# scheckmedia/centernet-uda

Hardware: AMD Instinct MI355X
Metric: images/sec CenterNet DLA-34 512x512 UDA step (entropy minimisation) (higher is better)
Workload: dtype f32; 1 GPU; configs[2]: DLA-34 + DCNv2, 512x512, per-GPU batch 16 source + 16 target, uda=entropy_minimization, Adam(lr 5e-5), random-init weights; global_batch=16, parallelism=dp1

## Files before the change

### centernet-uda_amd/csrc/conv.hip

```cpp
#include <stdlib.h>

#include <type_traits>
#include <algorithm>
#include "igemm.cuh"
#include "hconv.cuh"
#include "hwgrad.cuh"
#include "igemm_host.h"

namespace cnuda {
namespace {

struct ConvGeom {
    int B, C, H, W, Co, kh, kw, sh, sw, ph, pw, Ho, Wo;
};

struct ConvFwdParams {
    ConvGeom g;
    const float *x, *bias;
    float* y;
    float act_slope;
    const float* residual;
};
struct ConvFwdStatsParams : ConvFwdParams {
    float* stats;
// ... 1111 lines not shown
                                 : (ws ? "igemm_fwd_ws_kernel<%d, %s>" : "igemm_fwd_kernel<%d, %s>"), bm, Loader::name());
    if (matrix_mode() == 1) {
        float* A3 = const_cast<float*>(A) + (size_t)Kp * Mp;
        CNUDA_LAUNCH(split_a_kernel, dim3(stream_grid((long long)(Kp / 16) * 2 * Mp, 256)), dim3(256), 0, st, A,
                           reinterpret_cast<u32x4*>(A3), Kp, Mp);
        found = with_tile<32, 64, 128>(bm, [&](auto BM) {
            CNUDA_LAUNCH((igemm_fwd_kernel<BM(), Loader, true>), grid, block, 0, st, p, A3, Mp, Kp, M, N, n_tiles, m_tiles);
        });
    } else if (ws) {
        found = with_tile<64, 128>(bm, [&](auto BM) {
            CNUDA_LAUNCH((igemm_fwd_ws_kernel<BM(), Loader>), grid, block2, 0, st, p, A, Mp, Kp, M, N, n_tiles, m_tiles);
        });
    } else {
        found = with_tile<32, 64, 128>(bm, [&](auto BM) {
            CNUDA_LAUNCH((igemm_fwd_kernel<BM(), Loader>), grid, block, 0, st, p, A, Mp, Kp, M, N, n_tiles, m_tiles);
        });
    }
    CNUDA_REQUIRE(found, "%s: no igemm_fwd kernel instance for a %d-row tile", who, bm);
    return check_launch(who);
}

template <class Loader>
bool launch_wgrad_buf(const ConvPlan& q, const typename Loader::Params& p, float* slabs, float* bsl, hipStream_t st) {
    return q.wgrad_ws ? launch_wgrad<Loader, true, Tile<128, 128>, Tile<128, 64>, Tile<64, 128>, Tile<64, 64>>(q.wg, p, slabs, bsl, st)
                      : launch_wgrad<Loader, false, Tile<128, 128>, Tile<128, 64>, Tile<64, 128>, Tile<64, 64>, Tile<32, 128>>(q.wg, p, slabs, bsl, st);
}

using PlanQuery = bool (*)(const ConvGeom&, const ConvPlan&);
bool plan_cat_ok(const ConvGeom& g, const ConvPlan& q) {
    return q.fwd == FwdPath::Buf && q.dgrad == DgradPath::Buf && q.wgrad == WgradPath::Buf && ((g.H * g.W) & 3) == 0;
}
bool plan_rowquads_ok(const ConvGeom& g, const ConvPlan& q) { return g.Co % 4 == 0 && q.fwd != FwdPath::SmallC && q.fwd != FwdPath::BufSplitK && q.fwd_buf; }
bool plan_rowsig_ok(const ConvGeom& g, const ConvPlan& q) { return g.Co <= 32 && matrix_mode() == 0 && q.fwd != FwdPath::SmallC && q.fwd_buf && q.y_buf; }
int plan_query(PlanQuery ok, const char* who, int B, int C, int H, int W, int Co, int kh, int kw, int sh, int sw, int ph, int pw) {
    ConvGeom g;
    if (fill_geom(g, B, C, H, W, Co, kh, kw, sh, sw, ph, pw, who)) return 0;
    return ok(g, make_plan(g)) ? 1 : 0;
}

enum class ConvDir { Fwd = 0, Dgrad = 1, Wgrad = 2 };
struct ConvCall {
    const char* who;
    hipStream_t st;
    void* workspace;  size_t workspace_bytes;
    Carver cv;
    bool gemm_only = false;
    ConvGeom g;
    ConvPlan q;
    ConvCall(const char* who_, void* ws, size_t bytes, cnuda_stream_t stream)
        : who(who_), st((hipStream_t)stream), workspace(ws), workspace_bytes(bytes), cv(ws, bytes) {}
    FwdPath fwd() const { return gemm_only ? q.fwd_gemm : q.fwd; }
    DgradPath dgrad() const { return gemm_only ? q.dgrad_gemm : q.dgrad; }
    int open(ConvDir dir, bool gemm_only_, int B, int C, int H, int W, int Co, int kh, int kw, int sh, int sw, int ph, int pw,
             PlanQuery ok = nullptr, const char* unsupported = nullptr) {
        gemm_only = gemm_only_;
        const int bad = fill_geom(g, B, C, H, W, Co, kh, kw, sh, sw, ph, pw, who);
        if (!bad) q = make_plan(g);
        if (ok) CNUDA_REQUIRE(!bad && ok(g, q), "%s: %s", who, unsupported);
        if (bad) return bad;
        const bool lds_tiles[] = {fwd() == FwdPath::SmallC, dgrad() == DgradPath::SmallC, q.wgrad == WgradPath::SmallC};
        const size_t need[] = {q.fwd_bytes, q.dgrad_bytes, q.wgrad_bytes};
        CNUDA_REQUIRE(lds_tiles[(int)dir] || (workspace && workspace_bytes >= need[(int)dir]), "%s: workspace too small", who);
        return 0;
    }
    void rewind() { cv = Carver(workspace, workspace_bytes); }
    float* a_room(int Kp, int Mp) { return reinterpret_cast<float*>(cv.take<char>(ig_a_bytes(Kp, Mp))); }
// ... 182 lines not shown
}

extern "C" int cnuda_conv2d_forward_res(const float* x, const float* weight, const float* bias, const float* residual,
                                        float* y, int B, int C, int H, int W, int Cout, int kh, int kw, int sh, int sw,
                                        int ph, int pw, float act_slope, void* workspace, size_t workspace_bytes,
                                        cnuda_stream_t stream) {
    return cnuda_conv2d_forward_stats(x, weight, bias, residual, y, nullptr, B, C, H, W, Cout, kh, kw, sh, sw, ph, pw, act_slope,
                                      workspace, workspace_bytes, stream);
}

extern "C" int cnuda_conv2d_forward_stats(const float* x, const float* weight, const float* bias, const float* residual,
                                          float* y, float* stats, int B, int C, int H, int W, int Cout, int kh, int kw,
                                          int sh, int sw, int ph, int pw, float act_slope, void* workspace,
                                          size_t workspace_bytes, cnuda_stream_t stream) {
    CNUDA_REQUIRE(x && weight && y, "cnuda_conv2d_forward: null pointer");
    ConvCall c("cnuda_conv2d_forward", workspace, workspace_bytes, stream);
    if (int rc = c.open(ConvDir::Fwd, residual != nullptr, B, C, H, W, Cout, kh, kw, sh, sw, ph, pw)) return rc;
    CNUDA_REQUIRE(!stats || (!residual && act_slope < 0.0f && plan_stats_block(c.g, c.q, nullptr, nullptr) != 0),
                  "cnuda_conv2d_forward_stats: no statistics for this call (cnuda_conv2d_stats_block says which)");
    if (c.fwd() == FwdPath::SmallC)
        return smallc_forward(x, weight, bias, y, B, C, H, W, Cout, kh, kw, sh, ph, pw, act_slope, 0, workspace,
                              workspace_bytes, c.st, stats);
    ConvFwdParams p{c.g, x, bias, y, act_slope, residual};
    const float* A = c.pack(weight, c.fwd() == FwdPath::Halo ? PACK_HALO_FWD : PACK_FWD);
    switch (c.fwd()) {
        case FwdPath::Halo: return launch_hconv<HconvFwd>(c.q.bmf, p, x, C, c.g, A, c.q.Mpf, c.q.Kpf, Cout, c.q.Nf, c.st, c.who);
        case FwdPath::BufSplitK: case FwdPath::Buf:
            if (stats)
                return c.fwd_gemm<ConvFwdBufStatsLoader>(ConvFwdStatsParams{p, stats, c.q.Mpf}, A, "cnuda_conv2d_forward_stats");
            return c.fwd_gemm<ConvFwdBufLoader>(p, A, c.who, c.q.skf, c.splitk_slabs(c.q.skf, Cout, c.q.Nf));
        case FwdPath::PtrFast: return c.fwd_gemm<ConvFwdLoader<true>>(p, A, c.who);
        default: return c.fwd_gemm<ConvFwdLoader<false>>(p, A, c.who);
    }
}

extern "C" int cnuda_conv2d_cat_supported(const int* cs, int n, int B, int H, int W, int Cout) {
    const int C = cat_channels(cs, n);
    return C > 0 ? plan_query(plan_cat_ok, "cnuda_conv2d_cat_supported", B, C, H, W, Cout, 1, 1, 1, 1, 0, 0) : 0;
}

extern "C" int cnuda_conv2d_cat_forward(const float* const* xs, const int* cs, int n, const float* weight, const float* bias,
                                        float* y, float* stats, float act_slope, int B, int H, int W, int Cout,
                                        void* workspace, size_t workspace_bytes, cnuda_stream_t stream) {
    CNUDA_REQUIRE(weight && y, "cnuda_conv2d_cat_forward: null pointer");
    CNUDA_REQUIRE(!stats || act_slope < 0.0f, "cnuda_conv2d_cat_forward: statistics are those of the plain convolution");
    ConvCall c("cnuda_conv2d_cat_forward", workspace, workspace_bytes, stream);
    if (int rc = open_cat(c, ConvDir::Fwd, cs, n, B, H, W, Cout)) return rc;
    ConvFwdCatParams p{{{c.g, nullptr, bias, y, act_slope, nullptr}, stats, c.q.Mpf}, {}};
    if (int rc = fill_cat(p.cat, xs, cs, n, c.who)) return rc;
    return c.fwd_gemm<ConvFwdCatLoader>(p, c.pack(weight, PACK_FWD), c.who);
}

extern "C" int cnuda_conv2d_cat_backward_data(const float* grad_y, const float* weight, float* const* grad_xs,
                                              const float* const* adds, const float* const* add2s, const int* cs, int n,
                                              int B, int H, int W, int Cout, void* workspace, size_t workspace_bytes,
                                              cnuda_stream_t stream) {
    CNUDA_REQUIRE(grad_y && weight && grad_xs, "cnuda_conv2d_cat_backward_data: null pointer");
    ConvCall c("cnuda_conv2d_cat_backward_data", workspace, workspace_bytes, stream);
    if (int rc = open_cat(c, ConvDir::Dgrad, cs, n, B, H, W, Cout)) return rc;
    const float* A = c.pack(weight, PACK_DGRAD);
    ConvDgradCatParams p{{c.g, grad_y, nullptr, round_up(Cout, IG_BK), nullptr, nullptr}};
    for (int i = 0; i < CAT_MAX; ++i) {
        p.gxs[i] = i < n ? grad_xs[i] : nullptr;
        p.adds[i] = (i < n && adds) ? adds[i] : nullptr;
        p.add2s[i] = (i < n && add2s) ? add2s[i] : nullptr;
        if (!p.adds[i] && p.add2s[i]) { p.adds[i] = p.add2s[i]; p.add2s[i] = nullptr; }
// ... 179 lines not shown
```

### centernet-uda_amd/csrc/igemm.cuh

```cuda
#pragma once
#include <type_traits>
#include <utility>
#include "common.h"
#include "igemm_host.h"

namespace cnuda {

using f32x16 = __attribute__((ext_vector_type(16))) float;

constexpr int IG_BN = 128;
constexpr int IG_BK = 16;
constexpr int IG_KC = 16;
constexpr int IG_THREADS = 256;

template <int BM> struct IgTile;
template <> struct IgTile<128> { static constexpr int WM = 2, WN = 2, TM = 2, TN = 2; };
template <> struct IgTile<64>  { static constexpr int WM = 2, WN = 2, TM = 1, TN = 2; };
template <> struct IgTile<32>  { static constexpr int WM = 1, WN = 4, TM = 1, TN = 1; };

__device__ __forceinline__ int xcd_remap(int bid, int nwg) {
    constexpr int NX = 8;
    const int per = nwg / NX, rem = nwg % NX;
    const int x = bid % NX, q = bid / NX;
    const int start = x * per + (x < rem ? x : rem);
// ... 571 lines not shown
    }
    if constexpr (Loader::Out::kVec4) {
        if (Loader::Out::vec4_ok(p)) {
            ig_epilogue_vec4<BM, Loader>(p, smem + wid * IG_EPI_WAVE, acc, m0, n0, wm_off, wn_off, lane, M, N);
            return;
        }
    }
#pragma unroll
    for (int j = 0; j < T::TN; ++j) {
        const long long n = n0 + wn_off + j * 32 + (lane & 31);
        if (n >= N) continue;
        typename Loader::Out out(p, n);
#pragma unroll
        for (int i = 0; i < T::TM; ++i)
#pragma unroll
            for (int r = 0; r < 16; ++r) {
                const int m = m0 + wm_off + i * 32 + mfma_row(r, lane);
                if (m < M) out.store(p, m, acc[i][j][r]);
            }
    }
}

template <int BM, class Loader, int KC = IG_KC>
__global__ __launch_bounds__(2 * IG_THREADS, (BM == 128 ? 2 : 1)) void igemm_fwd_ws_kernel(
    typename Loader::Params p, const float* __restrict__ A, int Mp, int Kp, int M, long long N,
    int n_tiles, int m_tiles) {
    igemm_fwd_ws_body<BM, Loader, KC>(p, A, Mp, Kp, M, N, n_tiles, m_tiles);
}
template <int BM, class Loader, int KC = IG_KC>
__global__ __launch_bounds__(2 * IG_THREADS, (BM == 128 ? 2 : 1)) void igemm_fwd_ws_splitk_kernel(
    typename Loader::Params p, const float* __restrict__ A, int Mp, int Kp, int M, long long N,
    int n_tiles, int m_tiles, float* __restrict__ slab, int split_k) {
    igemm_fwd_ws_body<BM, Loader, KC, true>(p, A, Mp, Kp, M, N, n_tiles, m_tiles, slab, split_k);
}

template <int BMT, int LDA, class Loader, int KP>
__device__ __forceinline__ void ig_shortk_tile(const typename Loader::Params& p, float* __restrict__ As,
                                               const float* __restrict__ Bs, int m0, long long n0, int lane, int wid, int M,
                                               long long N) {
    using T = IgTile<BMT>;
    const int wm_off = (wid / T::WN) * (T::TM * 32), wn_off = (wid % T::WN) * (T::TN * 32);
    f32x16 acc[T::TM][T::TN];
    ig_zero(acc);
#pragma unroll
    for (int c = 0; c < KP / IG_KC; ++c)
        ig_mma_chunk<BMT, IG_KC, LDA>(As + c * IG_KC * LDA, Bs + c * IG_KC * IG_BN, acc, wm_off, wn_off, lane);
    if constexpr (IgHasQuads<typename Loader::Out>::value) {
        ig_epilogue_quads<BMT, Loader>(p, acc, m0, n0, wm_off, wn_off, lane, M, N);
        return;
    }
    __syncthreads();
    if constexpr (Loader::Out::kVec4) {
        if (Loader::Out::vec4_ok(p)) {
            ig_epilogue_vec4<BMT, Loader>(p, As + wid * IG_EPI_WAVE, acc, m0, n0, wm_off, wn_off, lane, M, N);
            return;
        }
    }
#pragma unroll
    for (int j = 0; j < T::TN; ++j) {
        const long long n = n0 + wn_off + j * 32 + (lane & 31);
        if (n >= N) continue;
        typename Loader::Out out(p, n);
#pragma unroll
        for (int i = 0; i < T::TM; ++i)
#pragma unroll
            for (int r = 0; r < 16; ++r) {
// ... 309 lines not shown
```

### centernet-uda_amd/hip_runtime/__init__.py

```python
import ctypes
import os
import threading
import weakref

import torch

_PKG_ROOT = os.path.dirname(os.path.dirname(os.path.abspath(__file__)))
LIB_PATH = os.path.join(_PKG_ROOT, 'libcenternet_uda_hip.so')
ABI_VERSION = 2

_lib = None
_lock = threading.Lock()
_workspaces = {}

c_int, c_size_t, c_void_p, c_float = ctypes.c_int, ctypes.c_size_t, ctypes.c_void_p, ctypes.c_float


def lib():
    global _lib
    if _lib is None:
        with _lock:
            if _lib is None:
                if not os.path.exists(LIB_PATH):
                    raise RuntimeError(
# ... 27 lines not shown
class _Sig:
    cnuda_decode_workspace_bytes = (c_size_t, [_I] * 5)
    cnuda_decode_set_max_bands = (_I, [_I])
    cnuda_decode_set_stage2_threads = (_I, [_I])
    cnuda_decode_detection = (_I, [_P] * 5 + [_I] * 8 + _WS)
    cnuda_nms = (_I, [_P, _P] + [_I] * 5 + [_P])
    cnuda_dcn_v2_workspace_bytes = (c_size_t, [_I] * 14)
    cnuda_dcn_v2_forward = (_I, [_P] * 6 + [_I] * 14 + _WS)
    cnuda_dcn_v2_backward = (_I, [_P] * 11 + [_I] * 14 + _WS)
    cnuda_dcn_v2_forward_cols = (_I, [_P] * 7 + [_I] * 14 + _WS)
    cnuda_dcn_v2_forward_act = (_I, [_P] * 7 + [_F] + [_I] * 14 + _WS)
    cnuda_dcn_v2_forward_stats = (_I, [_P] * 8 + [_I] * 16 + _WS)
    cnuda_dcn_v2_stats_block = (_I, [_I] * 14 + [_P])
    cnuda_dcn_v2_forward_om = (_I, [_P] * 7 + [_I] * 2 + [_F] + [_I] * 14 + _WS)
    cnuda_dcn_v2_backward_om = (_I, [_P] * 7 + [_I] + [_P] * 3 + [_I] * 14 + _WS)
    cnuda_dcn_v2_backward_cols = (_I, [_P] * 12 + [_I] * 14 + _WS)
    cnuda_dcn_v2_backward_acc = (_I, [_P] * 8 + [_I] + [_P] * 4 + [_I] * 14 + _WS)
    cnuda_dcn_v2_psroi_pooling_workspace_bytes = (c_size_t, [_I] * 4)
    cnuda_dcn_v2_psroi_pooling_forward = (_I, [_P] * 5 + [_I] * 6 + [_F] + [_I] * 5 + [_F, _I, _P])
    cnuda_dcn_v2_psroi_pooling_backward = (_I, [_P] * 6 + [_I, _P] + [_I] * 6 + [_F] + [_I] * 5 + [_F, _I] + _WS)
    cnuda_eval_workspace_bytes = (c_size_t, [_I, _I])
    cnuda_eval_box_spans = (_I, [_P, _I, _I, _I, _P, _P] + _WS)
    cnuda_eval_iou_rotated = (_I, [_P, _I, _I, _I, _LL, _P, _P, _I, _P] + _WS)
    cnuda_eval_iou_axis = (_I, [_P, _P, _P, _I, _I, _I, _LL, _P, _P])
    cnuda_eval_iou_quads = (_I, [_P, _P, _I, _I, _I, _LL, _P, _P, _P])
    cnuda_eval_match = (_I, [_P, _P, _I, _P, _P, _I, _I, _LL, _P, _I, _P, _P, _P, _P])
    cnuda_eval_match_flagged = (_I, [_P, _P, _I, _P, _P, _P, _I, _I, _LL, _P, _I, _P, _P, _P, _P])
    cnuda_eval_oks = (_I, [_P] * 6 + [_I, _P, _I, _I, _I, _LL, _P, _P, _P, _P])
    cnuda_conv2d_workspace_bytes = (c_size_t, [_I] * 11)
    cnuda_conv2d_forward = (_I, [_P] * 4 + [_I] * 11 + [_F] + _WS)
    cnuda_conv2d_forward_res = (_I, [_P] * 5 + [_I] * 11 + [_F] + _WS)
    cnuda_conv2d_rowsig_supported = (_I, [_I] * 11)
    cnuda_conv2d_forward_rowsig = (_I, [_P] * 4 + [_I] * 12 + _WS)
    cnuda_conv2d_rowquads_supported = (_I, [_I] * 11)
    cnuda_conv2d_cat_supported = (_I, [_P, _I, _I, _I, _I, _I])
    cnuda_conv2d_cat_forward = (_I, [_P, _P, _I, _P, _P, _P, _P, _F, _I, _I, _I, _I] + _WS)
    cnuda_conv2d_cat_backward_data = (_I, [_P, _P, _P, _P, _P, _P, _I, _I, _I, _I, _I] + _WS)
    cnuda_conv2d_cat_backward_weight = (_I, [_P, _P, _I, _P, _P, _I, _I, _I, _I] + _WS)
    cnuda_conv2d_forward_rowquads = (_I, [_P] * 3 + [_I] * 11 + _WS)
    cnuda_conv2d_backward_data = (_I, [_P] * 3 + [_I] * 11 + _WS)
    cnuda_conv2d_backward_data_add = (_I, [_P] * 5 + [_I] * 11 + _WS)
    cnuda_conv2d_stats_block = (_I, [_I] * 11 + [_P, _P])
    cnuda_conv2d_forward_stats = (_I, [_P] * 6 + [_I] * 11 + [_F] + _WS)
    cnuda_bn_train_forward_stats = (_I, [_P, _P, _LL, _I] + [_P] * 9 + [_F, _F, _I, _I, _I, _LL, _I] + _WS)
    cnuda_conv2d_backward_weight = (_I, [_P] * 4 + [_I] * 11 + _WS)
    cnuda_conv2d_norm_input_supported = (_I, [_I] * 11)
    cnuda_conv2d_forward_norm_input = (_I, [_P] * 5 + [_I] + [_P] * 4 + [_I] * 11 + [_F] + _WS)
    cnuda_conv2d_backward_weight_norm_input = (_I, [_P] * 5 + [_I] + [_P] * 3 + [_I] * 11 + _WS)
    cnuda_bn_workspace_bytes = (c_size_t, [_I, _I, _LL])
    cnuda_bn_plan = (_I, [_I, _I, _LL, _I] + [_P] * 4)
    cnuda_bn_train_forward = (_I, [_P] * 10 + [_F, _F, _I, _I, _I, _LL, _I] + _WS)
    cnuda_bn_eval_forward = (_I, [_P] * 7 + [_F, _I, _I, _I, _LL, _P])
    cnuda_bn_backward = (_I, [_P] * 11 + [_I, _I, _I, _LL, _I] + _WS)
    cnuda_maxpool2d_forward = (_I, [_P] * 2 + [_I] * 5 + [_P])
    cnuda_maxpool2d_backward = (_I, [_P] * 3 + [_I] * 5 + [_P])
    cnuda_maxpool2d_backward_acc = (_I, [_P] * 3 + [_I] * 6 + [_P])
    cnuda_maxpool2d_window_forward = (_I, [_P] * 2 + [_I] * 7 + [_P])
    cnuda_maxpool2d_window_backward = (_I, [_P] * 3 + [_I] * 7 + [_P])
    cnuda_dwconvt2d_forward = (_I, [_P] * 3 + [_I] * 7 + [_P])
    cnuda_dwconvt2d_add_forward = (_I, [_P] * 4 + [_I] * 7 + [_P])
    cnuda_dwconvt2d_workspace_bytes = (c_size_t, [_I] * 3)
    cnuda_dwconvt2d_backward = (_I, [_P] * 5 + [_I] * 7 + _WS)
    cnuda_dwconv2d_workspace_bytes = (c_size_t, [_I] * 3)
    cnuda_dwconv2d_forward = (_I, [_P] * 3 + [_I] * 7 + [_P])
    cnuda_dwconv2d_backward = (_I, [_P] * 5 + [_I] * 7 + _WS)
    cnuda_dwconv2d_same_workspace_bytes = (c_size_t, [_I] * 3)
# ... 457 lines not shown
```

### centernet-uda_amd/hip_runtime/nn.py

```python
import math

import torch
from torch import nn

from . import ops


def _pair(v):
    return tuple(v) if isinstance(v, (tuple, list)) else (v, v)


class Conv2d(nn.Module):

    def __init__(self, in_channels, out_channels, kernel_size, stride=1, padding=0, bias=True, act_slope=-1.0,
                 emit_stats=False):
        super().__init__()
        self.in_channels, self.out_channels = in_channels, out_channels
        self.kernel_size, self.stride, self.padding = _pair(kernel_size), _pair(stride), _pair(padding)
        self.act_slope = float(act_slope)
        self.emit_stats = bool(emit_stats)
        self.weight = nn.Parameter(torch.empty(out_channels, in_channels, *self.kernel_size))
        self.bias = nn.Parameter(torch.empty(out_channels)) if bias else None
        from . import PackToken
        self._pack_token = PackToken()
# ... 38 lines not shown
                                  defer_apply=self.defer_apply and self.training)


class MaxPool2d(nn.Module):
    def __init__(self, kernel_size, stride=None, padding=0):
        super().__init__()
        self.kernel_size = int(kernel_size)
        self.stride = self.kernel_size if stride is None else int(stride)
        self.padding = int(padding)

    def forward(self, x):
        return ops.max_pool2d(x, self.kernel_size, self.stride, self.padding)


class ConvTranspose2d(nn.Module):

    def __init__(self, in_channels, out_channels, kernel_size, stride=1, padding=0, output_padding=0):
        super().__init__()
        self.in_channels, self.out_channels = in_channels, out_channels
        self.kernel_size, self.stride = _pair(kernel_size), _pair(stride)
        self.padding, self.output_padding = _pair(padding), _pair(output_padding)
        self.weight = nn.Parameter(torch.empty(in_channels, out_channels, *self.kernel_size))
        bound = 1.0 / math.sqrt(out_channels * self.kernel_size[0] * self.kernel_size[1])
        with torch.no_grad():
            self.weight.uniform_(-bound, bound)

    def forward(self, x):
        return ops.conv_transpose2d(x, self.weight, self.stride, self.padding, self.output_padding)


class Head(nn.Sequential):

    def forward(self, x, lead=None):
        if len(self) == 3 and isinstance(self[0], Conv2d) and isinstance(self[2], Conv2d) \
                and not any(m._forward_hooks or m._forward_pre_hooks for m in self) \
                and (x.requires_grad or any(p.requires_grad for p in self.parameters())) \
                and ops.conv_act_conv1x1_supported(x, self[0], self[2]):
            return ops.conv_act_conv1x1(x, self[0], self[2], lead)
        return super().forward(x if lead is None else x[:lead])


class DepthwiseConvTranspose2d(nn.Module):

    def __init__(self, channels, kernel_size, stride, padding):
        super().__init__()
        self.channels, self.kernel_size, self.stride, self.padding = channels, kernel_size, stride, padding
        self.weight = nn.Parameter(torch.empty(channels, 1, kernel_size, kernel_size))
        with torch.no_grad():
            self.weight.uniform_(-1.0 / kernel_size, 1.0 / kernel_size)

    def forward(self, x, skip=None):
        return ops.depthwise_conv_transpose2d(x, self.weight, self.stride, self.padding, skip)


class DepthwiseConv2d(nn.Module):

    def __init__(self, channels, kernel_size, stride=1, padding=0):
        super().__init__()
        self.channels, self.kernel_size, self.stride, self.padding = channels, kernel_size, stride, padding
        self.in_channels = self.out_channels = channels
        self.weight = nn.Parameter(torch.empty(channels, 1, kernel_size, kernel_size))
        with torch.no_grad():
            self.weight.uniform_(-1.0 / kernel_size, 1.0 / kernel_size)

    def forward(self, x):
        return ops.depthwise_conv2d(x, self.weight, self.stride, self.padding)


class DepthwiseConv2dSame(nn.Module):

    def __init__(self, channels, kernel_size, stride=1, image_size=None):
# ... 98 lines not shown
```

### centernet-uda_amd/hip_runtime/ops.py

```python
import ctypes
import os

import torch
from torch.autograd import Function
from torch.autograd.function import once_differentiable

from . import check, f32c, lib, pack_stamp, prof_arm, ptr, require_gpu, stats_side_output, stream, workspace
from .arena import grad_sink
from .fanout import accumulate_in_place, accumulate_target, claim, first_writer, slot_of


def _pair(v):
    return tuple(v) if isinstance(v, (tuple, list)) else (v, v)


def _ws(nbytes, like):
    w = workspace(nbytes, like.device)
    return ptr(w), w.numel()


def _param_grad(param, needed=True):
    if not needed or param is None:
        return None, None
    v = grad_sink(param)
# ... 106 lines not shown
    if bias is None or not lib().cnuda_conv2d_rowsig_supported(*g):
        return None
    return _Conv2d.apply(x, weight, bias, stride, padding, -1.0, pack_token, None, None, int(sig_from))


EPILOGUE_STATS = True


def with_bn_stats(emit, call):
    if not (emit and EPILOGUE_STATS):
        return call(None)
    box = []
    y = call(box)
    if box:
        y._cnuda_bn_stats = box[0]
    return y


def conv2d(x, weight, bias=None, stride=1, padding=0, act_slope=-1.0, pack_token=0, emit_stats=False):
    norm = getattr(x, '_cnuda_deferred_bn', None)
    if norm is not None:
        g = _conv_geom(x, weight, stride, padding)
        if not lib().cnuda_conv2d_norm_input_supported(*g):
            raise RuntimeError("conv2d: the input is a deferred BatchNorm output, but no apply-on-load kernel takes this "
                               "convolution (cnuda_conv2d_norm_input_supported); ask batch_norm_act to apply it")
    return with_bn_stats(emit_stats, lambda box: _Conv2d.apply(x, weight, bias, stride, padding, float(act_slope), pack_token,
                                                               box, norm, None))


HEAD_SPARSE = os.environ.get('CNUDA_HEAD_SPARSE', '1') != '0'
HEAD_SPARSE_RATIO = 40


def _mark_sparse_rows(grad, ind, mask, B, M, HW):
    grad._cnuda_sparse_rows = (ind, mask, B, M, HW, grad._version)


def _sparse_rows_of(gy, B, HW):
    mark = gy.__dict__.pop('_cnuda_sparse_rows', None)
    if mark is None or mark[5] != gy._version or mark[2] != B or mark[4] != HW or not gy.is_contiguous():
        return None
    return mark[0], mark[1], mark[3]


class _ConvActConv1x1(Function):

    @staticmethod
    def forward(ctx, x, w1, b1, w2, b2, padding, act_slope, token1, token2, lead=None):
        require_gpu(x, w1, b1, w2, b2)
        ctx.slot, ctx.full = slot_of(x), None
        if lead is not None and lead < x.shape[0]:
            ctx.full = x.shape
            x = f32c(x)[:lead]
        x, w1, w2 = f32c(x), f32c(w1), f32c(w2)
        b1 = None if b1 is None else f32c(b1)
        b2 = None if b2 is None else f32c(b2)
        g1 = _conv_geom(x, w1, 1, padding)
        hidden = _conv_forward(g1, x, w1, b1, act_slope, token1)
        g2 = _conv_geom(hidden, w2, 1, 0)
        y = _conv_forward(g2, hidden, w2, b2, -1.0, token2)
        ctx.g1, ctx.g2, ctx.act_slope, ctx.token1 = g1, g2, float(act_slope), token1
        ctx.has_b1, ctx.has_b2 = b1 is not None, b2 is not None
        ctx.save_for_backward(x, w1, b1, w2, b2, hidden)
        return y

    @staticmethod
    @once_differentiable
    def backward(ctx, gy):
        x, w1, b1, w2, b2, hidden = ctx.saved_tensors
        g1, g2 = ctx.g1, ctx.g2
        L = lib()
        gy = f32c(gy)
        if gy.data_ptr() % 16:
            gy = gy.clone()
        B, Ch, Co = g1[0], g1[4], g2[4]
        rows = _sparse_rows_of(gy, B, hidden.shape[2] * hidden.shape[3])
        if rows is not None and HEAD_SPARSE:
            sparse = _ConvActConv1x1._backward_sparse(ctx, gy, *rows)
            if sparse is not None:
                return sparse
        gx = gw1 = gb1 = gw2 = gb2 = None
        if ctx.needs_input_grad[3] or (ctx.has_b2 and ctx.needs_input_grad[4]):
            gw2, gb2 = _conv_wgrad(g2, hidden, gy, w2, b2)
        gh = torch.empty_like(hidden)
        check(L.cnuda_conv1x1_backward_data_act(ptr(gy), ptr(w2), ptr(hidden), ptr(gh), B, Co, Ch, hidden.shape[2] * hidden.shape[3],
                                                ctx.act_slope, stream()), 'conv1x1_backward_data_act')
        if ctx.needs_input_grad[0]:
            slot = ctx.slot
            if ctx.full is None:
                gx, addend, addend2 = accumulate_target(slot, x)
                part = gx
            elif (gx := accumulate_in_place(slot)) is not None:
                part = addend = gx[:B]
# ... 20 lines not shown
        gx = part = None
        if ctx.needs_input_grad[0]:
            slot = ctx.slot
            if slot is not None and slot.buf is not None and not slot.owned:
                return None
            gx = accumulate_in_place(slot)
            if gx is None:
                gx = claim(slot, torch.zeros(ctx.full or x.shape, dtype=torch.float32, device=x.device))
            part = gx[:B]
        gw1 = gb1 = gw2 = gb2 = gw1_buf = gb1_buf = gw2_buf = gb2_buf = None
        if ctx.needs_input_grad[1] or (ctx.has_b1 and ctx.needs_input_grad[2]):
            (gw1_buf, gw1), (gb1_buf, gb1) = _param_grad(w1), _param_grad(b1)
        if ctx.needs_input_grad[3] or (ctx.has_b2 and ctx.needs_input_grad[4]):
            (gw2_buf, gw2), (gb2_buf, gb2) = _param_grad(w2), _param_grad(b2)
        wp, wn = _ws(L.cnuda_head_backward_sparse_workspace_bytes(B, M, C, H, W, Ch, Co, kh, kw), x)
        check(L.cnuda_head_backward_sparse(ptr(gy), ptr(ind), ptr(mask), ptr(x), ptr(hidden), ptr(w1), ptr(w2), ptr(part),
                                           ptr(gw1_buf), ptr(gb1_buf), ptr(gw2_buf), ptr(gb2_buf), B, M, C, H, W, Ch, Co, kh, kw,
                                           ctx.act_slope, wp, wn, stream()), 'head_backward_sparse')
        return gx, gw1, gb1, gw2, gb2, None, None, None, None, None


def conv_act_conv1x1_supported(x, conv, last):
    if not (torch.is_grad_enabled() and x.is_cuda and x.dim() == 4):
        return False
    (kh, kw), (ph, pw) = conv.kernel_size, conv.padding
    hw = (x.shape[2] + 2 * ph - kh + 1) * (x.shape[3] + 2 * pw - kw + 1)
    return (conv.act_slope >= 0 and conv.stride == (1, 1) and last.kernel_size == (1, 1) and last.stride == (1, 1)
            and last.padding == (0, 0) and last.act_slope < 0 and 1 <= last.out_channels <= 8 and hw > 0 and hw % 4 == 0)


def conv_act_conv1x1(x, conv, last, lead=None):
    return _ConvActConv1x1.apply(x, conv.weight, conv.bias, last.weight, last.bias, conv.padding, conv.act_slope,
                                 conv._pack_token, last._pack_token, lead)


def conv2d_infer(x, weight, bias=None, stride=1, padding=0, act_slope=-1.0, residual=None, pack_token=0,
                 pack_version=None):
    require_gpu(x, weight, bias, residual)
    x, weight = f32c(x.detach()), f32c(weight.detach())
    bias = None if bias is None else f32c(bias.detach())
    g = _conv_geom(x, weight, stride, padding)
    B, C, H, W, Co, kh, kw, sh, sw, ph, pw = g
    Ho, Wo = (H + 2 * ph - kh) // sh + 1, (W + 2 * pw - kw) // sw + 1
    if residual is not None:
        residual = f32c(residual.detach())
        if tuple(residual.shape) != (B, Co, Ho, Wo):
            raise RuntimeError("conv2d_infer: residual %s does not match the output %s"
                               % (tuple(residual.shape), (B, Co, Ho, Wo)))
    return _conv_forward(g, x, weight, bias, act_slope, pack_token, pack_version, residual=residual)


class _ConvTranspose2d(Function):

    @staticmethod
    def forward(ctx, x, weight, stride, padding, output_padding):
        require_gpu(x, weight)
        x, weight = f32c(x), f32c(weight)
        B, Ci, H, W = x.shape
        if weight.shape[0] != Ci:
            raise RuntimeError("conv_transpose2d: input has %d channels, weight expects %d" % (Ci, weight.shape[0]))
        Co, kh, kw = weight.shape[1], weight.shape[2], weight.shape[3]
        (sh, sw), (ph, pw), (oph, opw) = _pair(stride), _pair(padding), _pair(output_padding)
        Ho, Wo = (H - 1) * sh - 2 * ph + kh + oph, (W - 1) * sw - 2 * pw + kw + opw
        g = (B, Co, Ho, Wo, Ci, kh, kw, sh, sw, ph, pw)
        if (Ho + 2 * ph - kh) // sh + 1 != H or (Wo + 2 * pw - kw) // sw + 1 != W:
            raise RuntimeError("conv_transpose2d: output_padding %s inconsistent with stride %s" %
# ... 1283 lines not shown
```

### include/centernet_uda_hip.h

```cpp
#ifndef CENTERNET_UDA_HIP_H
#define CENTERNET_UDA_HIP_H

#include <stddef.h>
#include <stdint.h>

#ifdef __cplusplus
extern "C" {
#endif

#define CNUDA_ERR_INVALID_ARGUMENT (-1)
#define CNUDA_ABI_VERSION 2

typedef void* cnuda_stream_t;

int cnuda_abi_version(void);
const char* cnuda_last_error(void);

int cnuda_set_matrix_mode(int mode);
int cnuda_get_matrix_mode(void);

int cnuda_pack_cache_attach(void* arena, size_t bytes);
int cnuda_pack_stamp(unsigned long long token, unsigned long long version);
size_t cnuda_pack_cache_used(void);
unsigned long long cnuda_pack_cache_fills(void);
// ... 117 lines not shown
                           void* workspace, size_t workspace_bytes, cnuda_stream_t stream);
int cnuda_eval_iou_axis(const float* det_boxes, const float* gt_boxes, const int* groups, int num_groups,
                        int num_det, int num_gt, long long num_pairs, double* iou, cnuda_stream_t stream);
int cnuda_eval_iou_quads(const float* quads, const int* groups, int num_groups, int num_det, int num_gt,
                         long long num_pairs, double* iou, double* area, cnuda_stream_t stream);
int cnuda_eval_match(const double* iou, const int* groups, int num_groups, const double* det_area,
                     const double* gt_area, int num_det, int num_gt, long long num_pairs,
                     const double* thresholds, int num_thresholds, const double* area_ranges,
                     unsigned* det_bits, unsigned char* gt_ignore, cnuda_stream_t stream);
int cnuda_eval_match_flagged(const double* iou, const int* groups, int num_groups, const double* det_area,
                             const double* gt_area, const unsigned char* gt_flags, int num_det, int num_gt,
                             long long num_pairs, const double* thresholds, int num_thresholds,
                             const double* area_ranges, unsigned* det_bits, unsigned char* gt_ignore,
                             cnuda_stream_t stream);
int cnuda_eval_oks(const float* det_kps, const float* gt_kps, const unsigned char* gt_vis, const double* gt_area,
                   const float* gt_box, const double* sigmas, int num_joints, const int* groups, int num_groups,
                   int num_det, int num_gt, long long num_pairs, double* oks, double* det_area,
                   unsigned char* gt_flags, cnuda_stream_t stream);

size_t cnuda_conv2d_workspace_bytes(int B, int C, int H, int W, int Cout, int kh, int kw,
                                    int sh, int sw, int ph, int pw);
int cnuda_conv2d_forward(const float* x, const float* weight, const float* bias, float* y,
                         int B, int C, int H, int W, int Cout, int kh, int kw,
                         int sh, int sw, int ph, int pw, float act_slope,
                         void* workspace, size_t workspace_bytes, cnuda_stream_t stream);
int cnuda_conv2d_forward_res(const float* x, const float* weight, const float* bias, const float* residual, float* y,
                             int B, int C, int H, int W, int Cout, int kh, int kw,
                             int sh, int sw, int ph, int pw, float act_slope,
                             void* workspace, size_t workspace_bytes, cnuda_stream_t stream);
int cnuda_conv2d_rowsig_supported(int B, int C, int H, int W, int Cout, int kh, int kw, int sh, int sw, int ph, int pw);
int cnuda_conv2d_forward_rowsig(const float* x, const float* weight, const float* bias, float* y, int sig_from,
                                int B, int C, int H, int W, int Cout, int kh, int kw, int sh, int sw, int ph, int pw,
                                void* workspace, size_t workspace_bytes, cnuda_stream_t stream);
int cnuda_conv2d_cat_supported(const int* cs, int n, int B, int H, int W, int Cout);
int cnuda_conv2d_cat_forward(const float* const* xs, const int* cs, int n, const float* weight, const float* bias ,
                             float* y, float* stats, float act_slope ,
                             int B, int H, int W, int Cout, void* workspace, size_t workspace_bytes, cnuda_stream_t stream);
int cnuda_conv2d_cat_backward_data(const float* grad_y, const float* weight, float* const* grad_xs, const float* const* adds,
                                   const float* const* add2s, const int* cs, int n, int B, int H, int W, int Cout,
                                   void* workspace, size_t workspace_bytes, cnuda_stream_t stream);
int cnuda_conv2d_cat_backward_weight(const float* const* xs, const int* cs, int n, const float* grad_y, float* grad_weight,
                                     int B, int H, int W, int Cout, void* workspace, size_t workspace_bytes,
                                     cnuda_stream_t stream);
int cnuda_conv2d_rowquads_supported(int B, int C, int H, int W, int Cout, int kh, int kw, int sh, int sw, int ph, int pw);
int cnuda_conv2d_forward_rowquads(const float* x, const float* weight, float* y,
                                  int B, int C, int H, int W, int Cout, int kh, int kw, int sh, int sw, int ph, int pw,
                                  void* workspace, size_t workspace_bytes, cnuda_stream_t stream);
int cnuda_conv2d_stats_block(int B, int C, int H, int W, int Cout, int kh, int kw, int sh, int sw, int ph, int pw, int* rows,
                             int* blocks_per_image );
int cnuda_conv2d_forward_stats(const float* x, const float* weight, const float* bias, const float* residual, float* y,
                               float* stats, int B, int C, int H, int W, int Cout, int kh, int kw,
                               int sh, int sw, int ph, int pw, float act_slope,
                               void* workspace, size_t workspace_bytes, cnuda_stream_t stream);
int cnuda_conv2d_backward_data(const float* grad_y, const float* weight, float* grad_x,
                               int B, int C, int H, int W, int Cout, int kh, int kw,
                               int sh, int sw, int ph, int pw,
                               void* workspace, size_t workspace_bytes, cnuda_stream_t stream);
int cnuda_conv2d_norm_input_supported(int B, int C, int H, int W, int Cout, int kh, int kw, int sh, int sw, int ph, int pw);
int cnuda_conv2d_forward_norm_input(const float* x, const float* mean, const float* invstd, const float* gamma,
                                    const float* beta, int imgs_per_group, const float* weight, const float* bias, float* y,
                                    float* stats, int B, int C, int H, int W, int Cout, int kh, int kw, int sh, int sw, int ph,
                                    int pw, float act_slope, void* workspace, size_t workspace_bytes, cnuda_stream_t stream);
int cnuda_conv2d_backward_weight_norm_input(const float* x, const float* mean, const float* invstd, const float* gamma,
                                            const float* beta, int imgs_per_group, const float* grad_y, float* grad_weight,
                                            float* grad_bias, int B, int C, int H, int W, int Cout, int kh, int kw, int sh,
                                            int sw, int ph, int pw, void* workspace, size_t workspace_bytes,
// ... 268 lines not shown
```

Before: 219.1 images/sec.

## Fuse head 3x3 conv, activation and 1x1 conv into one kernel

Adds a wave-specialised implicit-GEMM kernel that computes the head's first convolution, applies bias and activation, and reduces the hidden channels against the 1x1 output weights in registers. The output is written directly, and the hidden map is stored only when training needs it. This removes the separate 1x1 convolution launch and its reread of the hidden tensor. The catch is a more complex kernel that is limited to Ch<=256 and Co<=8, and that recomputes across all M tiles within a single block per pixel tile.

```diff
diff --git a/centernet-uda_amd/csrc/conv.hip b/centernet-uda_amd/csrc/conv.hip
--- a/centernet-uda_amd/csrc/conv.hip
+++ b/centernet-uda_amd/csrc/conv.hip
@@ -1167,6 +1167,11 @@
 }
 bool plan_rowquads_ok(const ConvGeom& g, const ConvPlan& q) { return g.Co % 4 == 0 && q.fwd != FwdPath::SmallC && q.fwd != FwdPath::BufSplitK && q.fwd_buf; }
 bool plan_rowsig_ok(const ConvGeom& g, const ConvPlan& q) { return g.Co <= 32 && matrix_mode() == 0 && q.fwd != FwdPath::SmallC && q.fwd_buf && q.y_buf; }
+bool plan_head_ok(const ConvGeom& g, const ConvPlan& q) {
+    return matrix_mode() == 0 && wave_specialised() && q.fwd == FwdPath::Buf && q.y_buf && g.sh == 1 && g.sw == 1 &&
+           g.kh == g.kw && (g.kh == 1 || g.kh == 3) && g.Ho == g.H && g.Wo == g.W && g.Co % 128 == 0 && g.Co <= IG_HEAD_MAXM &&
+           ((g.H * g.W) & 3) == 0;
+}
 int plan_query(PlanQuery ok, const char* who, int B, int C, int H, int W, int Co, int kh, int kw, int sh, int sw, int ph, int pw) {
     ConvGeom g;
     if (fill_geom(g, B, C, H, W, Co, kh, kw, sh, sw, ph, pw, who)) return 0;
@@ -1415,6 +1420,33 @@
         case FwdPath::PtrFast: return c.fwd_gemm<ConvFwdLoader<true>>(p, A, c.who);
         default: return c.fwd_gemm<ConvFwdLoader<false>>(p, A, c.who);
     }
+}
+
+extern "C" int cnuda_conv2d_head_supported(int B, int C, int H, int W, int Ch, int kh, int kw, int ph, int pw, int Cout) {
+    if (Cout < 1 || Cout > IG_HEAD_MAXCO) return 0;
+    return plan_query(plan_head_ok, "cnuda_conv2d_head_supported", B, C, H, W, Ch, kh, kw, 1, 1, ph, pw);
+}
+
+extern "C" int cnuda_conv2d_forward_head(const float* x, const float* w1, const float* b1, float act_slope, const float* w2,
+                                         const float* b2, float* hidden, float* y, int B, int C, int H, int W, int Ch, int kh,
+                                         int kw, int ph, int pw, int Cout, void* workspace, size_t workspace_bytes,
+                                         cnuda_stream_t stream) {
+    CNUDA_REQUIRE(x && w1 && w2 && y, "cnuda_conv2d_forward_head: null pointer");
+    CNUDA_REQUIRE(Cout >= 1 && Cout <= IG_HEAD_MAXCO, "cnuda_conv2d_forward_head: 1 .. %d outputs (cnuda_conv2d_head_supported)", IG_HEAD_MAXCO);
+    ConvCall c("cnuda_conv2d_forward_head", workspace, workspace_bytes, stream);
+    if (int rc = c.open(ConvDir::Fwd, false, B, C, H, W, Ch, kh, kw, 1, 1, ph, pw, plan_head_ok,
+                        "geometry without a head epilogue (cnuda_conv2d_head_supported)"))
+        return rc;
+    CNUDA_REQUIRE(c.q.Nf < (1ll << 31) - IG_BN, "cnuda_conv2d_forward_head: more than 2^31 pixels per call");
+    const ConvFwdParams p{c.g, x, b1, hidden, act_slope, nullptr};
+    const IgHeadTail tail{w2, b2, y, Cout, H * W};
+    const float* A = c.pack(w1, PACK_FWD);
+    const int n_tiles = ceil_div(c.q.Nf, IG_BN), Mp = round_up(Ch, 128);
+    ProfScope prof(c.st);
+    prof.name("igemm_fwd_ws_head_kernel<%s>", ConvFwdBufLoader::name());
+    CNUDA_LAUNCH((igemm_fwd_ws_head_kernel<ConvFwdBufLoader>), dim3(n_tiles), dim3(2 * IG_THREADS), 0, c.st, p, tail, A, Mp,
+                 c.q.Kpf, Ch, c.q.Nf, n_tiles);
+    return check_launch(c.who);
 }
 
 extern "C" int cnuda_conv2d_cat_supported(const int* cs, int n, int B, int H, int W, int Cout) {
diff --git a/centernet-uda_amd/csrc/igemm.cuh b/centernet-uda_amd/csrc/igemm.cuh
--- a/centernet-uda_amd/csrc/igemm.cuh
+++ b/centernet-uda_amd/csrc/igemm.cuh
@@ -627,6 +627,123 @@
     typename Loader::Params p, const float* __restrict__ A, int Mp, int Kp, int M, long long N,
     int n_tiles, int m_tiles, float* __restrict__ slab, int split_k) {
     igemm_fwd_ws_body<BM, Loader, KC, true>(p, A, Mp, Kp, M, N, n_tiles, m_tiles, slab, split_k);
+}
+
+constexpr int IG_HEAD_MAXCO = 8, IG_HEAD_MAXM = 256;
+struct IgHeadTail {
+    const float *w2, *b2;
+    float* y;
+    int Co, HW;
+};
+template <class Loader>
+__global__ __launch_bounds__(2 * IG_THREADS, 2) void igemm_fwd_ws_head_kernel(
+    typename Loader::Params p, IgHeadTail h, const float* __restrict__ A, int Mp, int Kp, int M, long long N, int n_tiles) {
+    constexpr int BM = 128, KC = IG_KC;
+    using T = IgTile<BM>;
+    constexpr int LDS_AB = 2 * KC * BM + 2 * KC * IG_BN;
+    static_assert(LDS_AB >= 4 * IG_EPI_WAVE + 2 * IG_HEAD_MAXCO * IG_BN, "the operand buffers hold the staging tiles and the partials");
+    __shared__ __attribute__((aligned(16))) float smem[LDS_AB];
+    __shared__ __attribute__((aligned(16))) float w2s[IG_HEAD_MAXCO * IG_HEAD_MAXM];
+    __shared__ __attribute__((aligned(16))) float b1s[IG_HEAD_MAXM];
+    float (*As)[KC * BM] = reinterpret_cast<float (*)[KC * BM]>(smem);
+    float (*Bs)[KC * IG_BN] = reinterpret_cast<float (*)[KC * IG_BN]>(smem + 2 * KC * BM);
+    const bool producer = threadIdx.x >= IG_THREADS;
+    const int tid = threadIdx.x & (IG_THREADS - 1), lane = tid & 63, wid = tid >> 6;
+    const long long n0 = (long long)xcd_remap(blockIdx.x, n_tiles) * IG_BN;
+    const int m_tiles = Mp / BM;
+    if (producer) {
+        for (int e = tid; e < h.Co * M; e += IG_THREADS) w2s[e] = h.w2[e];
+        for (int e = tid; e < M; e += IG_THREADS) b1s[e] = p.bias ? p.bias[e] : 0.0f;
+        const int nl = tid & (IG_BN - 1);
+        for (int mt = 0; mt < m_tiles; ++mt) {
+            Loader ld(p, n0 + nl, n0 + nl < N);
+            IgFwdStager<BM, Loader, KC, false> stg(ld, A, Mp, Kp, mt * BM, tid);
+            stg.load(0);
+            if (mt > 0) __syncthreads();
+            stg.store(As[0], Bs[0]);
+            if (KC < Kp) stg.load(KC);
+            __syncthreads();
+            int c1 = 0;
+            for (int k0 = 0; k0 < Kp; k0 += KC) {
+                if (k0 + KC < Kp) {
+                    stg.store(As[c1 ^ 1], Bs[c1 ^ 1]);
+                    if (k0 + 2 * KC < Kp) stg.load(k0 + 2 * KC);
+                }
+                __syncthreads();
+                c1 ^= 1;
+            }
+        }
+        __syncthreads();
+        return;
+    }
+    const int wm_off = (wid / T::WN) * (T::TM * 32), wn_off = (wid % T::WN) * (T::TN * 32);
+    const bool has_b1 = p.bias != nullptr;
+    float part[T::TN][IG_HEAD_MAXCO];
+#pragma unroll
+    for (int j = 0; j < T::TN; ++j)
+#pragma unroll
+        for (int o = 0; o < IG_HEAD_MAXCO; ++o) part[j][o] = 0.0f;
+    for (int mt = 0; mt < m_tiles; ++mt) {
+        const int m0 = mt * BM;
+        f32x16 acc[T::TM][T::TN];
+        ig_zero(acc);
+        if (mt > 0) __syncthreads();
+        __syncthreads();
+        int cur = 0;
+        for (int k0 = 0; k0 < Kp; k0 += KC) {
+            ig_mma_chunk<BM, KC>(As[cur], Bs[cur], acc, wm_off, wn_off, lane);
+            __syncthreads();
+            cur ^= 1;
+        }
+        if (p.y) ig_epilogue_vec4<BM, Loader>(p, smem + wid * IG_EPI_WAVE, acc, m0, n0, wm_off, wn_off, lane, M, N);
+#pragma unroll
+        for (int i = 0; i < T::TM; ++i)
+#pragma unroll
+            for (int q = 0; q < 4; ++q) {
+                const int m = m0 + wm_off + i * 32 + 8 * q + 4 * (lane >> 5);
+                const f32x4 bq = *reinterpret_cast<const f32x4*>(b1s + m);
+                float hv[T::TN][4];
+#pragma unroll
+                for (int j = 0; j < T::TN; ++j)
+#pragma unroll
+                    for (int e = 0; e < 4; ++e) {
+                        float v = acc[i][j][4 * q + e];
+                        if (has_b1) v += bq[e];
+                        if (p.act_slope >= 0.0f && v < 0.0f) v *= p.act_slope;
+                        hv[j][e] = v;
+                    }
+#pragma unroll
+                for (int o = 0; o < IG_HEAD_MAXCO; ++o) {
+                    if (o < h.Co) {
+                        const f32x4 wq = *reinterpret_cast<const f32x4*>(w2s + o * M + m);
+#pragma unroll
+                        for (int j = 0; j < T::TN; ++j)
+#pragma unroll
+                            for (int e = 0; e < 4; ++e) part[j][o] = __builtin_fmaf(wq[e], hv[j][e], part[j][o]);
+                    }
+                }
+            }
+    }
+    float* xs = smem + 4 * IG_EPI_WAVE;
+#pragma unroll
+    for (int j = 0; j < T::TN; ++j)
+#pragma unroll
+        for (int o = 0; o < IG_HEAD_MAXCO; ++o) {
+            if (o < h.Co) {
+                const float s = part[j][o] + __shfl_xor(part[j][o], 32, 64);
+                if (lane < 32) xs[((wid / T::WN) * IG_HEAD_MAXCO + o) * IG_BN + wn_off + j * 32 + lane] = s;
+            }
+        }
+    __syncthreads();
+    const int px = tid & (IG_BN - 1);
+    const long long n = n0 + px;
+    if (n >= N) return;
+    const int b = (int)(n / h.HW), pp = (int)(n - (long long)b * h.HW);
+    for (int o = tid >> 7; o < h.Co; o += 2) {
+        float v = xs[o * IG_BN + px] + xs[(IG_HEAD_MAXCO + o) * IG_BN + px];
+        if (h.b2) v += h.b2[o];
+        h.y[((size_t)b * h.Co + o) * h.HW + pp] = v;
+    }
 }
 
 template <int BMT, int LDA, class Loader, int KP>
diff --git a/centernet-uda_amd/hip_runtime/__init__.py b/centernet-uda_amd/hip_runtime/__init__.py
--- a/centernet-uda_amd/hip_runtime/__init__.py
+++ b/centernet-uda_amd/hip_runtime/__init__.py
@@ -83,6 +83,8 @@
     cnuda_conv2d_forward_res = (_I, [_P] * 5 + [_I] * 11 + [_F] + _WS)
     cnuda_conv2d_rowsig_supported = (_I, [_I] * 11)
     cnuda_conv2d_forward_rowsig = (_I, [_P] * 4 + [_I] * 12 + _WS)
+    cnuda_conv2d_head_supported = (_I, [_I] * 10)
+    cnuda_conv2d_forward_head = (_I, [_P] * 3 + [_F] + [_P] * 4 + [_I] * 10 + _WS)
     cnuda_conv2d_rowquads_supported = (_I, [_I] * 11)
     cnuda_conv2d_cat_supported = (_I, [_P, _I, _I, _I, _I, _I])
     cnuda_conv2d_cat_forward = (_I, [_P, _P, _I, _P, _P, _P, _P, _F, _I, _I, _I, _I] + _WS)
diff --git a/centernet-uda_amd/hip_runtime/nn.py b/centernet-uda_amd/hip_runtime/nn.py
--- a/centernet-uda_amd/hip_runtime/nn.py
+++ b/centernet-uda_amd/hip_runtime/nn.py
@@ -94,11 +94,15 @@
 class Head(nn.Sequential):
 
     def forward(self, x, lead=None):
-        if len(self) == 3 and isinstance(self[0], Conv2d) and isinstance(self[2], Conv2d) \
-                and not any(m._forward_hooks or m._forward_pre_hooks for m in self) \
-                and (x.requires_grad or any(p.requires_grad for p in self.parameters())) \
+        pair = len(self) == 3 and isinstance(self[0], Conv2d) and isinstance(self[2], Conv2d) \
+            and not any(m._forward_hooks or m._forward_pre_hooks for m in self)
+        if pair and (x.requires_grad or any(p.requires_grad for p in self.parameters())) \
                 and ops.conv_act_conv1x1_supported(x, self[0], self[2]):
             return ops.conv_act_conv1x1(x, self[0], self[2], lead)
+        if pair and type(self[1]) is Slot:
+            y = ops.conv_act_conv1x1_infer(x, self[0], self[2], lead)
+            if y is not None:
+                return y
         return super().forward(x if lead is None else x[:lead])
 
 
diff --git a/centernet-uda_amd/hip_runtime/ops.py b/centernet-uda_amd/hip_runtime/ops.py
--- a/centernet-uda_amd/hip_runtime/ops.py
+++ b/centernet-uda_amd/hip_runtime/ops.py
@@ -162,6 +162,28 @@
 HEAD_SPARSE_RATIO = 40
 
 
+HEAD_FUSED = os.environ.get('CNUDA_HEAD_FUSED', '1') != '0'
+
+
+def _head_forward(x, w1, b1, w2, b2, padding, act_slope, token1, keep_hidden):
+    if not HEAD_FUSED or w2.dim() != 4 or w2.shape[2:] != (1, 1) or w2.shape[1] != w1.shape[0]:
+        return None
+    g1 = _conv_geom(x, w1, 1, padding)
+    B, C, H, W, Ch, kh, kw, _, _, ph, pw = g1
+    Co = w2.shape[0]
+    L = lib()
+    if not L.cnuda_conv2d_head_supported(B, C, H, W, Ch, kh, kw, ph, pw, Co):
+        return None
+    hidden = torch.empty((B, Ch, H, W), dtype=torch.float32, device=x.device) if keep_hidden else None
+    y = torch.empty((B, Co, H, W), dtype=torch.float32, device=x.device)
+    wp, wn = _ws(L.cnuda_conv2d_workspace_bytes(*g1), x)
+    prof_arm('conv_fwd', B, C, H, W, Ch, kh, kw, H, W)
+    with pack_stamp(token1, w1):
+        check(L.cnuda_conv2d_forward_head(ptr(x), ptr(w1), ptr(b1), float(act_slope), ptr(w2), ptr(b2), ptr(hidden), ptr(y),
+                                          B, C, H, W, Ch, kh, kw, ph, pw, Co, wp, wn, stream()), 'conv2d_forward_head')
+    return hidden, y
+
+
 def _mark_sparse_rows(grad, ind, mask, B, M, HW):
     grad._cnuda_sparse_rows = (ind, mask, B, M, HW, grad._version)
 
@@ -186,9 +208,14 @@
         b1 = None if b1 is None else f32c(b1)
         b2 = None if b2 is None else f32c(b2)
         g1 = _conv_geom(x, w1, 1, padding)
-        hidden = _conv_forward(g1, x, w1, b1, act_slope, token1)
-        g2 = _conv_geom(hidden, w2, 1, 0)
-        y = _conv_forward(g2, hidden, w2, b2, -1.0, token2)
+        fused = _head_forward(x, w1, b1, w2, b2, padding, act_slope, token1, keep_hidden=True)
+        if fused is not None:
+            hidden, y = fused
+            g2 = _conv_geom(hidden, w2, 1, 0)
+        else:
+            hidden = _conv_forward(g1, x, w1, b1, act_slope, token1)
+            g2 = _conv_geom(hidden, w2, 1, 0)
+            y = _conv_forward(g2, hidden, w2, b2, -1.0, token2)
         ctx.g1, ctx.g2, ctx.act_slope, ctx.token1 = g1, g2, float(act_slope), token1
         ctx.has_b1, ctx.has_b2 = b1 is not None, b2 is not None
         ctx.save_for_backward(x, w1, b1, w2, b2, hidden)
@@ -275,6 +302,23 @@
 def conv_act_conv1x1(x, conv, last, lead=None):
     return _ConvActConv1x1.apply(x, conv.weight, conv.bias, last.weight, last.bias, conv.padding, conv.act_slope,
                                  conv._pack_token, last._pack_token, lead)
+
+
+def conv_act_conv1x1_infer(x, conv, last, lead=None):
+    needs_tape = torch.is_grad_enabled() and (x.requires_grad or any(p.requires_grad for m in (conv, last) for p in m.parameters()))
+    if needs_tape or not (x.is_cuda and x.dim() == 4 and x.dtype == torch.float32):
+        return None
+    if not (conv.act_slope >= 0 and conv.stride == (1, 1) and last.kernel_size == (1, 1) and last.stride == (1, 1)
+            and last.padding == (0, 0) and last.act_slope < 0):
+        return None
+    x = x.detach()
+    if lead is not None:
+        x = x[:lead]
+    b1 = None if conv.bias is None else f32c(conv.bias)
+    b2 = None if last.bias is None else f32c(last.bias)
+    fused = _head_forward(f32c(x), f32c(conv.weight), b1, f32c(last.weight), b2, conv.padding,
+                          conv.act_slope, conv._pack_token, keep_hidden=False)
+    return None if fused is None else fused[1]
 
 
 def conv2d_infer(x, weight, bias=None, stride=1, padding=0, act_slope=-1.0, residual=None, pack_token=0,
diff --git a/include/centernet_uda_hip.h b/include/centernet_uda_hip.h
--- a/include/centernet_uda_hip.h
+++ b/include/centernet_uda_hip.h
@@ -173,6 +173,10 @@
 int cnuda_conv2d_forward_rowsig(const float* x, const float* weight, const float* bias, float* y, int sig_from,
                                 int B, int C, int H, int W, int Cout, int kh, int kw, int sh, int sw, int ph, int pw,
                                 void* workspace, size_t workspace_bytes, cnuda_stream_t stream);
+int cnuda_conv2d_head_supported(int B, int C, int H, int W, int Ch, int kh, int kw, int ph, int pw, int Cout);
+int cnuda_conv2d_forward_head(const float* x, const float* w1, const float* b1, float act_slope, const float* w2,
+                              const float* b2, float* hidden, float* y, int B, int C, int H, int W, int Ch, int kh, int kw,
+                              int ph, int pw, int Cout, void* workspace, size_t workspace_bytes, cnuda_stream_t stream);
 int cnuda_conv2d_cat_supported(const int* cs, int n, int B, int H, int W, int Cout);
 int cnuda_conv2d_cat_forward(const float* const* xs, const int* cs, int n, const float* weight, const float* bias ,
                              float* y, float* stats, float act_slope ,
```

Measured after the change: 218.3 images/sec. No clear change (-0.3%).
